# MiraPurkrabek/ProbPose_code

Hardware: AMD Instinct MI355X
Metric: person-crops/sec @ 256x192 bs64 (higher is better)
Workload: dtype f16x3; 1 GPU; ProbPose-small (ViT-S 12x384, 12 heads x 32) bs64 random 256x192 uint8 crops per GPU, flip_test=True, seeded random-init weights: preprocess -> backbone x2 passes -> ProbMapHead (heatmap branch + Sparsemax + 4 towers) -> ProbMap decode -> results in pinned host memory; crops_per_gpu=64, global_batch=64, parallelism=dp1, steps_in_flight=2

## Files before the change

include/probpose_mi355x.h:

```cpp
#ifndef PROBPOSE_MI355X_H_
#define PROBPOSE_MI355X_H_

#include <stddef.h>
#include <stdint.h>

#ifdef __cplusplus
extern "C" {
#endif

#define PP_ABI_VERSION 4


enum {
    PP_OK = 0,
    PP_ERR_INVALID_ARG = -1,
    PP_ERR_UNSUPPORTED = -2,
    PP_ERR_HIP = -3,
    PP_ERR_WORKSPACE = -4
};

#define PP_MAX_RADIUS 9
#define PP_MAX_TAPS (2 * PP_MAX_RADIUS + 1)

int pp_abi_version(void);
// ... 168 lines not shown
                         const float* head_b, float* logits_phased, int B, int H, int W, int Cin, int Cout, int K, void* stream);

int pp_probmap_head_decode_phased(const float* logits, const float* logits_flip, const int32_t* flip_indices,
                                  const double* taps, const int32_t* radius, int B, int K, int H, int W, double in_w,
                                  double in_h, float temperature, float normalize, float* avg_out, float* conv_out,
                                  float* locs, double* keypoints, float* scores, void* stream);

#define PP_DECODE_LOGITS 1
#define PP_DECODE_PHASED 2
#define PP_DECODE_SHIFT_HEATMAP 4
int pp_probmap_decode_flags(const float* maps, const float* maps_flip, const int32_t* flip_indices, const double* taps,
                            const int32_t* radius, int B, int K, int H, int W, double in_w, double in_h, float temperature,
                            float normalize, float* avg_out, float* conv_out, float* locs, double* keypoints, float* scores,
                            int flags, void* stream);

int pp_udp_heatmap_decode(const float* maps, const float* maps_flip, const int32_t* flip_indices, int B, int K, int H, int W,
                          double in_w, double in_h, int blur_kernel_size, float* avg_out, float* locs, double* keypoints,
                          float* scores, int flags, void* stream);

int pp_expmax_heatmap_decode(const float* maps, const float* maps_flip, const int32_t* flip_indices, const double* taps,
                             const int32_t* radius, int B, int K, int H, int W, double in_w, double in_h, float* avg_out,
                             float* conv_out, float* locs, double* keypoints, float* scores, int flags, void* stream);

int pp_argmax_probmap_decode(const float* logits, const float* logits_flip, const int32_t* flip_indices, int B, int K, int H, int W,
                             double in_w, double in_h, float temperature, float normalize, int blur_kernel_size, float* avg_out,
                             float* locs, double* keypoints, float* scores, int flags, void* stream);

int pp_conv3x3_splitk(int prec, const void* act_nhwc, const void* weight, float* partials, int B, int H, int W, int Cin,
                      int Cout, int groups, long long stride_act_g, long long stride_w_g, int ksplit, void* stream);
int pp_sum_maxpool_relu_nhwc(const float* partials, int nsplit, long long split_stride, const float* bias,
                             int images_per_group, void* out, int out_bf16, int N, int H, int W, int C, int ph, int pw,
                             void* stream);

long long pp_winograd_scratch_bytes(int B, int H, int W, int Cin);
int pp_conv3x3_winograd_maxpool_relu(const void* act_nhwc, const void* u_packed, const float* bias, void* v_scratch,
                                     void* out_pooled, int B, int H, int W, int Cin, int Cout, int pool_h, int pool_w, int groups,
                                     void* stream);

int pp_tower_final(const void* feat, int feat_bf16, const float* w, const float* bias,
                   const int32_t* flip_indices, float* out, int B, int passes, int C, int K, float err_div,
                   void* stream);

int pp_extended_oks(const double* gt_kpts, const double* gt_bbox, const double* gt_area, const double* dt_kpts,
                    const double* sigmas, const int* gt_visibilities, int G, int D, int K, int n_vis,
                    double confidence_thr, double padding, int use_area, int original, double* out, void* stream);

int pp_pack_records(const double* keypoints, const float* scores, const float* scalars, double* records, int n, void* stream);

int pp_revert_heatmaps_max(const float* heatmaps, const double* inverse_maps, float* out, int n, int K, int hm_h, int hm_w,
                           int img_h, int img_w, void* stream);

int pp_heatmap_posterior(float* heatmaps, const float* presence, double* scratch, int K, int H, int W, void* stream);

int pp_exoks_cells(const double* gt_kpts, const double* gt_bbox, const double* gt_area, const double* dt_kpts,
                   const double* sigmas, const int* gt_visibilities, const int* cell_gt_off, const int* cell_dt_off,
                   const long long* cell_out_off, int n_cells, int K, int n_vis, double confidence_thr, double padding,
                   int use_area, int original, double* out, void* stream);

int pp_exoks_match(const double* ious, const int* cell_gt_off, const int* cell_dt_off, const long long* cell_iou_off,
                   const unsigned char* gt_ignore, const unsigned char* gt_iscrowd, const double* gt_area,
                   const double* gt_bbox, const double* dt_area, const double* dt_bbox, const double* area_rng,
                   const double* iou_thrs, int n_cells, int max_gt_per_cell, int N_gt, int N_dt, int L, int A, int T,
                   int match_by_bbox, int* dt_match, unsigned char* dt_ignore, int* gt_match,
                   unsigned char* gt_ignore_out, double* sim_sum, int* sim_cnt, void* stream);

int pp_exmap_accumulate(const int* dt_match, const unsigned char* dt_ignore, const unsigned char* gt_ignore,
// ... 25 lines not shown
```

probpose_code_amd/_lib.py:

```python
import ctypes
import os
from ctypes import c_char_p, c_double, c_float, c_int, c_longlong, c_void_p

import torch

_HERE = os.path.dirname(os.path.abspath(__file__))
LIB_NAME = "libprobpose_mi355x.so"
LIB_PATH = os.path.join(_HERE, LIB_NAME)

PP_OK = 0
PP_ERR_INVALID_ARG = -1
PP_ERR_UNSUPPORTED = -2
PP_ERR_HIP = -3
PP_ERR_WORKSPACE = -4
PP_MAX_RADIUS = 9
PP_MAX_TAPS = 2 * PP_MAX_RADIUS + 1


class ProbPoseLibraryError(RuntimeError):

    def __init__(self, fn, status, message):
        super().__init__(f"{fn} failed with {status}: {message}")
        self.status = status

# ... 63 lines not shown
        c_int,
        [c_int, _P, _P, _P, _P, c_int, _P, c_int, c_int, c_int, c_int, c_int, c_int, c_int, c_int, c_int, c_float, _P],
    ),
    "pp_gemm_residual_layernorm": (
        c_int,
        [c_int, _P, _P, _P, _P, c_int, _P, _P, _P, c_float, _P, c_int, c_int, c_int, c_int, c_int, c_int, _P],
    ),
    "pp_gemm_residual_layernorm_ws": (
        c_int,
        [c_int, _P, _P, _P, _P, c_int, _P, _P, _P, c_float, _P, c_int, c_int, c_int, c_int, c_int, c_int, c_float, _P],
    ),
    "pp_mlp_residual_layernorm": (c_int, [_P, _P, _P, _P, _P, _P, _P, _P, _P, c_float, _P, c_int, c_int, c_int, _P]),
    "pp_proj_mlp_residual_layernorm": (
        c_int, [_P, _P, _P, _P, _P, _P, _P, _P, _P, _P, _P, _P, _P, c_float, _P, _P, _P, _P, c_int, c_int, c_int, _P]),
    "pp_vit_layer": (
        c_int, [_P, c_int, c_int, c_float, _P, _P, _P, _P, _P, _P, _P, _P, _P, _P, _P, _P, c_float, _P, _P, _P, _P, c_int, c_int,
                c_int, _P]),
    "pp_ffn_split_packed_bytes": (c_longlong, [c_int, c_int]),
    "pp_ffn_split_pack_weights": (c_int, [_P, _P, _P, c_int, c_int, _P]),
    "pp_ffn_split_residual_layernorm": (c_int, [_P, _P, _P, _P, _P, _P, _P, _P, c_float, _P, c_int, c_int, c_int, _P]),
    "pp_ffn_split_residual_layernorm_ws": (c_int, [_P, _P, _P, _P, _P, _P, _P, _P, c_float, _P, c_int, c_int, c_int, c_float, c_float, _P]),
    "pp_qkv_attention_split": (c_int, [_P, _P, _P, _P, c_int, c_int, c_int, c_int, c_float, _P]),
    "pp_qkv_attention_split_ws": (c_int, [_P, _P, _P, _P, c_int, c_int, c_int, c_int, c_float, c_float, _P]),
    "pp_qkv_attention_split_folded": (c_int, [_P] * 5 + [c_int] * 4 + [c_float, c_float, _P]),
    "pp_proj_split_packed_bytes": (c_longlong, [c_int]),
    "pp_proj_split_pack_weights": (c_int, [_P, _P, c_int, _P]),
    "pp_proj_ffn_split_residual_layernorm": (
        c_int, [_P, _P, _P, _P, _P, _P, _P, _P, _P, _P, _P, _P, _P, c_float, _P, c_int, c_int, c_int, _P]),
    "pp_proj_ffn_split_residual_layernorm_ws": (
        c_int, [_P, _P, _P, _P, _P, _P, _P, _P, _P, _P, _P, _P, _P, c_float, _P, c_int, c_int, c_int, c_float, c_float, c_float, _P]),
    "pp_proj_ffn_split_folded": (
        c_int, [_P] * 10 + [c_int, _P, c_int, _P, _P, _P, c_float, _P, _P, c_int, c_int, c_int, c_float, c_float, c_float, _P]),
    "pp_conv3x3_splitk": (c_int, [c_int, _P, _P, _P, c_int, c_int, c_int, c_int, c_int, c_int, c_longlong, c_longlong, c_int, _P]),
    "pp_sum_maxpool_relu_nhwc": (c_int, [_P, c_int, c_longlong, _P, c_int, _P, c_int, c_int, c_int, c_int, c_int, c_int, c_int, _P]),
    "pp_warp_affine_u8": (c_int, [_P, c_int, c_int, c_int, _P, _P, c_int, c_int, c_int, _P]),
    "pp_warp_affine_u8_batch": (c_int, [_P, _P, c_int, _P, _P, c_int, c_int, _P, c_int, c_int, c_int, _P]),
    "pp_extended_oks": (
        c_int, [_P, _P, _P, _P, _P, _P, c_int, c_int, c_int, c_int, c_double, c_double, c_int, c_int, _P, _P]),
    "pp_pack_records": (c_int, [_P, _P, _P, _P, c_int, _P]),
    "pp_revert_heatmaps_max": (c_int, [_P, _P, _P] + [c_int] * 6 + [_P]),
    "pp_heatmap_posterior": (c_int, [_P, _P, _P, c_int, c_int, c_int, _P]),
    "pp_exoks_cells": (
        c_int, [_P] * 9 + [c_int, c_int, c_int, c_double, c_double, c_int, c_int, _P, _P]),
    "pp_exoks_match": (
        c_int, [_P] * 12 + [c_int] * 8 + [_P] * 7),
    "pp_exmap_accumulate": (
        c_int, [_P] * 6 + [c_int] * 7 + [_P] * 5),
    "pp_conv_gemm": (
        c_int,
        [c_int, c_int, _P, _P, _P, _P, c_int, c_int, c_int, c_int, c_int, c_int, c_int, c_int,
         c_longlong, c_longlong, c_longlong, c_longlong, c_int, c_int, c_int, _P],
    ),
    "pp_attention": (c_int, [c_int, _P, _P, c_int, c_int, c_int, c_int, c_float, _P]),
    "pp_preproc_im2col": (c_int, [c_int, _P, c_int, _P, c_int, c_int, c_int, c_int, c_int, c_int, _P, _P, c_int, _P]),
    "pp_layernorm": (c_int, [_P, _P, _P, _P, c_int, c_int, c_float, c_int, _P]),
    "pp_maxpool_relu_nhwc": (c_int, [_P, c_int, _P, c_int, c_int, c_int, c_int, c_int, c_int, c_int, _P]),
    "pp_conv3x3_maxpool_relu": (c_int, [c_int, _P, _P, _P, _P, _P] + [c_int] * 8 + [c_longlong] * 3 + [c_int, _P]),
    "pp_winograd_scratch_bytes": (c_longlong, [c_int] * 4),
    "pp_conv3x3_winograd_maxpool_relu": (c_int, [_P] * 5 + [c_int] * 8 + [_P]),
    "pp_tower_final": (c_int, [_P, c_int, _P, _P, _P, _P, c_int, c_int, c_int, c_int, c_float, _P]),
    "pp_parea_scratch_bytes": (c_longlong, [c_int, c_int, c_int]),
    "pp_parea_thresholds": (c_int, [_P, c_int, c_int, c_int, _P, _P, _P, _P]),
    "pp_parea_compose": (c_int, [_P, c_int, c_int, c_int, c_int, _P, c_int, _P, _P, _P, c_int, _P, c_int, c_int, _P]),
    "pp_draw_poses": (
        c_int, [_P, c_int, c_int, _P, _P, _P, c_int, c_int, _P, _P, _P, c_int, c_double, c_float, c_float, c_float, _P, _P]),
    "pp_resize_bilinear_u8": (c_int, [_P, c_int, c_int, _P, c_int, c_int, _P]),
# ... 104 lines not shown
```

probpose_code_amd/csrc/pp_gemm.h:

```cpp
#pragma once
#include "pp_common.h"

namespace pp {

enum { G_LINEAR = 0, G_CONV3 = 1, G_DECONV = 2 };
enum { ACT_NONE = 0, ACT_GELU = 1, ACT_RELU = 2 };

struct GemmParams {
    const void* A;
    const void* W;
    void* C;
    const float* bias;
    const float* residual;
    int M, N, K;
    int lda, ldw, ldc;
    int H, Wd, Cin;
    int py, px;
    int act;
    int out_bf16;
    int gather;
    int res_mod;
    int ldres;
    const void* head_w;
    const float* head_b;
    float* head_out;
    int head_n;
    int ksplit;
    int groups;
    int pool_h, pool_w;
    int tap_inner;
    int tile_order;
    int planar_P;
    unsigned a_bytes, w_bytes;
    float w_inv = 1.0f;
    long long strideA_z, strideW_z, strideC_z, strideBias_z;
};

int gemm(const GemmParams& p, int prec, int groups, hipStream_t s);

bool panel_gemm_supported(const GemmParams& p, int prec, int groups);
int panel_gemm(const GemmParams& p, int groups, hipStream_t s);

bool conv_halo_supported(const GemmParams& p, int prec, int groups);
int conv_halo(const GemmParams& p, int groups, hipStream_t s);

bool panel_split_supported(const GemmParams& p, int prec, int groups);
int panel_split_gemm(const GemmParams& p, int prec, int groups, hipStream_t s);

bool linear_dma_supported(const GemmParams& p, int prec, int groups);
int linear_dma_gemm(const GemmParams& p, hipStream_t s);

}
```

probpose_code_amd/csrc/pp_gemm.hip:

```cpp
#include "pp_common.h"
#include "pp_gemm.h"
#include "pp_split.h"

#include <cstdlib>

namespace pp {

typedef __bf16 bf16x8 __attribute__((ext_vector_type(8)));
typedef __bf16 bf16x4 __attribute__((ext_vector_type(4)));
typedef float f32x4 __attribute__((ext_vector_type(4)));
typedef unsigned int u32x4 __attribute__((ext_vector_type(4)));
typedef __attribute__((address_space(3))) void* lds_ptr_t;

constexpr int BM = 128, BN = 128;
constexpr int GEMM_THREADS = 256;
constexpr int ROW_BYTES = 128;
constexpr int TILE_BYTES = BM * ROW_BYTES;
constexpr int BUF_BYTES = 2 * TILE_BYTES;
constexpr unsigned OOB_OFFSET = 0x7ffffff0u;

template <typename T>
struct Prec;
template <>
struct Prec<__bf16> {
// ... 496 lines not shown
}

extern "C" int pp_conv3x3_splitk(int prec, const void* act_nhwc, const void* weight, float* partials, int B, int H, int W,
                                 int Cin, int Cout, int groups, long long stride_act_g, long long stride_w_g, int ksplit,
                                 void* stream) {
    using namespace pp;
    PP_REQUIRE(act_nhwc && weight && partials, PP_ERR_INVALID_ARG, "pp_conv3x3_splitk: NULL argument");
    PP_REQUIRE(groups >= 1 && B > 0 && H > 0 && W > 0 && Cin > 0 && Cout > 0, PP_ERR_INVALID_ARG, "pp_conv3x3_splitk: bad shape");
    PP_REQUIRE(ksplit >= 1 && ksplit <= 16 && (ksplit == 1 || ksplit == 3 || ksplit == 9 || Cin % (32 * ksplit) == 0), PP_ERR_UNSUPPORTED,
               "pp_conv3x3_splitk: ksplit must be 1, 3 or 9 (whole taps), or a count of channel ranges (Cin % (32 ksplit) == 0, split-fp16 wide-tile kernel)");
    GemmParams p{};
    p.A = act_nhwc; p.W = weight; p.C = partials; p.bias = nullptr; p.residual = nullptr;
    p.M = B * H * W; p.N = Cout;
    p.K = 9 * Cin / ksplit;
    p.lda = Cin; p.ldw = 9 * Cin; p.ldc = Cout;
    p.H = H; p.Wd = W; p.Cin = Cin;
    p.act = ACT_NONE; p.out_bf16 = 0; p.gather = G_CONV3; p.ldres = Cout;
    p.ksplit = ksplit;
    const size_t esz = prec == PP_PREC_BF16 ? 2 : 4;
    const size_t ab = (size_t)B * H * W * Cin * esz, wb = (size_t)Cout * 9 * Cin * esz;
    PP_REQUIRE(ab < 0x7ffffff0u && wb < 0x7ffffff0u, PP_ERR_UNSUPPORTED, "pp_conv3x3_splitk: operands must be smaller than 2 GiB");
    p.a_bytes = (unsigned)ab; p.w_bytes = (unsigned)wb;
    p.strideA_z = stride_act_g; p.strideW_z = stride_w_g; p.strideC_z = (long long)p.M * Cout; p.strideBias_z = 0;
    if (ksplit != 1 && ksplit != 3 && ksplit != 9) {
        PP_REQUIRE(panel_enabled() && panel_split_supported(p, prec, groups * ksplit), PP_ERR_UNSUPPORTED,
                   "pp_conv3x3_splitk: this slice count is a channel-range split, built for the split-fp16 wide-tile kernel only (use pp_conv3x3_splitk_slices)");
        return panel_split_gemm(p, prec, groups * ksplit, reinterpret_cast<hipStream_t>(stream));
    }
    if (panel_enabled() && panel_gemm_supported(p, prec, groups * ksplit))
        return panel_gemm(p, groups * ksplit, reinterpret_cast<hipStream_t>(stream));
    return gemm(p, prec, groups * ksplit, reinterpret_cast<hipStream_t>(stream));
}

extern "C" int pp_deconv_head(const void* act_nhwc, const void* weight, const float* bias, const void* head_w,
                              const float* head_b, float* logits_phased, int B, int H, int W, int Cin, int Cout, int K,
                              void* stream) {
    using namespace pp;
    PP_REQUIRE(act_nhwc && weight && head_w && head_b && logits_phased, PP_ERR_INVALID_ARG, "pp_deconv_head: NULL argument");
    PP_REQUIRE(B > 0 && H > 0 && W > 0 && Cin > 0, PP_ERR_INVALID_ARG, "pp_deconv_head: bad shape");
    PP_REQUIRE(Cout == 256 && K >= 1 && K <= 28 && Cin % 32 == 0 && (4 * Cin) % 128 == 0 && (H * W) % 4 == 0, PP_ERR_UNSUPPORTED,
               "pp_deconv_head: built for 256 deconvolution channels, at most 28 output maps, Cin % 32 == 0, H*W % 4 == 0");
    GemmParams p{};
    p.A = act_nhwc; p.W = weight; p.C = logits_phased; p.bias = bias; p.residual = nullptr;
    p.M = B * H * W; p.N = Cout; p.K = 4 * Cin;
    p.lda = Cin; p.ldw = p.K; p.ldc = Cout;
    p.H = H; p.Wd = W; p.Cin = Cin; p.py = -1; p.px = -1;
    p.act = ACT_RELU; p.out_bf16 = 1; p.gather = G_DECONV; p.ldres = Cout;
    p.head_w = head_w; p.head_b = head_b; p.head_out = logits_phased; p.head_n = K;
    const size_t ab = (size_t)B * H * W * Cin * 2, wb = (size_t)Cout * p.K * 2;
    PP_REQUIRE(ab < 0x7ffffff0u && wb < 0x7ffffff0u, PP_ERR_UNSUPPORTED, "pp_deconv_head: operands must be smaller than 2 GiB");
    p.a_bytes = (unsigned)ab; p.w_bytes = (unsigned)wb;
    p.strideA_z = 0; p.strideW_z = (long long)Cout * 4 * Cin; p.strideC_z = 0; p.strideBias_z = 0;
    return panel_gemm(p, 4, reinterpret_cast<hipStream_t>(stream));
}

extern "C" int pp_deconv_head_split(const void* act_nhwc, const void* weight, const float* bias, const void* head_w_packed,
                                    const float* head_b, float* logits_phased, int B, int H, int W, int Cin, int Cout, int K,
                                    void* stream) {
    using namespace pp;
    PP_REQUIRE(act_nhwc && weight && head_w_packed && head_b && logits_phased, PP_ERR_INVALID_ARG, "pp_deconv_head_split: NULL argument");
    PP_REQUIRE(B > 0 && H > 0 && W > 0 && Cin > 0, PP_ERR_INVALID_ARG, "pp_deconv_head_split: bad shape");
    PP_REQUIRE(Cout == 256 && K >= 1 && K <= 28 && Cin % 32 == 0, PP_ERR_UNSUPPORTED,
               "pp_deconv_head_split: built for 256 deconvolution channels, at most 28 output maps, Cin % 32 == 0");
    GemmParams p{};
    p.A = act_nhwc; p.W = weight; p.C = logits_phased; p.bias = bias; p.residual = nullptr;
    p.M = B * H * W; p.N = Cout; p.K = 4 * Cin;
// ... 13 lines not shown
```

probpose_code_amd/engine.py:

```python
import math
import os
import warnings
from typing import Dict, Optional, Sequence

import numpy as np
import ctypes

import torch

from . import _lib
from .codecs import oks_kernel_taps
from .weights import PackedWeights, from_split, pack, to_split

PREC = {"bf16": 0, "f32": 1, "f16x3": 2}
_DTYPE = {"bf16": torch.bfloat16, "f32": torch.float32, "f16x3": torch.float32}
_FMT = {"bf16": 1, "f32": 0, "f16x3": 2}
ACT_NONE, ACT_GELU, ACT_RELU = 0, 1, 2
CONV3X3, DECONV = 1, 2


PLAN_DEFAULTS = dict(fuse_mlp=True, fuse_proj=True, fuse_qkv=True, split_k=True, fuse_attn=True, fuse_head=True, fuse_resln=None,
                     fuse_pool=True, fuse_qkv_attn=True, winograd=True, ln_fold=True, small_plan=True, head_two_streams=True)
SMALL_PLAN_ROWS_BELOW = 6912


def plan_from_env() -> Dict[str, object]:
    out: Dict[str, object] = {}
    for k in PLAN_DEFAULTS:
        v = os.environ.get("PP_" + k.upper())
        if v in ("0", "1"):
            out[k] = v == "1"
    return out


class _CapturedGraph:

    def __init__(self, graph, static_in, out, events, side_stream, raw_stream):
        self.graph, self.static_in, self.out, self.events, self.side_stream, self.raw_stream = graph, static_in, out, events, side_stream, raw_stream

    def release(self):
        if self.graph is None and self.raw_stream is None:
            return
        try:
            if torch.cuda.is_available():
                torch.cuda.synchronize()
        except Exception:
            pass
        self.graph = None
        self.out = self.static_in = None
        self.events = []
        self.side_stream = None
        raw, self.raw_stream = self.raw_stream, None
        if raw:
            try:
                _lib.lib.pp_stream_destroy(ctypes.c_void_p(raw))
# ... 113 lines not shown
        self.ln_fold = bool(precision == "f16x3" and pl["ln_fold"] and not self._proj_packed and not self._ffn_packed
                            and self.w.has("l0.fc1.wf") and self.E % 192 == 0 and self.w.ffn_dims % 192 == 0)
        self.ln_fold_fused = bool(precision == "f16x3" and pl["ln_fold"] and self.fuse_qkv_attn and self._proj_packed and self.w.has("l1.qkv.wf")
                                  and (self.w.ffn_dims // 128) % 2 == 0 and self.w.num_layers >= 2)
        if precision == "f16x3":
            if self.fuse_qkv_attn and self._proj_packed:
                self.layer_plan = "two launches per layer (pp_qkv_attention_split + pp_proj_ffn_split_residual_layernorm)"
                if self.ln_fold_fused:
                    self.layer_plan += "; ln1 of layers 1 .. L - 1 folded into the qkv projection (pp_proj_ffn_split_folded -> pp_qkv_attention_split_folded)"
            elif self._proj_packed:
                self.layer_plan = "three launches per layer (pp_gemm qkv + pp_attention + pp_proj_ffn_split_residual_layernorm)"
            else:
                self.layer_plan = "generic (pp_gemm / pp_attention / pp_layernorm per layer)"
                if self.ln_fold:
                    self.layer_plan += ("; from the row count at which the twelve-wave Linear kernel engages: LayerNorm folded into the Linear "
                                        "layers (pp_linear_ln_folded x4 + pp_attention per layer, residual stream in the operand format)")
                if self.hd == 80:
                    self.layer_plan += "; attention at head dim 80: pp_attention_hd80.hip (the q . k contraction zero-padded to 96 on chip)"
                if self._small_at(1):
                    self.layer_plan += (f"; batches of fewer than {SMALL_PLAN_ROWS_BELOW} token rows: the small-batch plan (pp_skinny_linear x4 + "
                                        "pp_attention per layer, LayerNorm in the Linear launches)")
                elif self.small_plan and self.E > 1024:
                    self.layer_plan += f"; no small-batch plan at E = {self.E} (pp_skinny_linear's LayerNorm tail ends at 1024 columns): this plan at every batch size"
            if pl["fuse_qkv_attn"] and not self.fuse_qkv_attn and self.E == 384 and self.hd == 32:
                warnings.warn(
                    f"ProbPoseEngine: {self.Np}-token sequences ({img_size[0]}x{img_size[1]} input) miss the fused qkv + attention kernel, "
                    f"which is built for 192 tokens (256x192); this model runs {self.layer_plan}", RuntimeWarning, stacklevel=2)
        else:
            self.layer_plan = "bf16 / f32 plan"
        self.winograd = (precision == "f16x3" and pl["winograd"] and self.w.has("tower0.wino")
                         and _lib.lib.pp_winograd_scratch_bytes(1, self.Hp, self.Wp, self.E) > 0)
        if self.w.has("tower0.wino") and not self.winograd:
            self.w.t.pop("tower0.wino")
        self._logits_phased = False
        self._head_stream: Optional[torch.cuda.Stream] = None
        self._capture_events: list = []
        self._eager_events: dict = {}
        self.profile: Optional[Dict[str, list]] = None
        self.stage_hook = None
        self.pools = ((4, 3), (2, 2), (2, 2))
        hs, ws_ = self.Hp, self.Wp
        self.tower_hw = []
        for ph, pw_ in self.pools if self.head_kind == "probmap" else ():
            self.tower_hw.append((hs, ws_))
            hs, ws_ = hs // ph, ws_ // pw_
        if self.head_kind == "probmap" and (hs, ws_) != (1, 1):
            raise ValueError(
                f"scalar towers reduce the {self.Hp}x{self.Wp} feature map to {hs}x{ws_}; the reference "
                "reshapes them to (B, 1, K) (probmap_head.py:780-783), which needs 1x1"
            )

    def ksplit(self, nb: int, th: int, tw: int) -> int:
        return int(_lib.lib.pp_conv3x3_splitk_slices(self.prec, int(nb), int(th), int(tw), self.E, self.E, 4))

    def _workspace(self, B: int, passes: int, slot: int = 0) -> Dict[str, torch.Tensor]:
        self._check_options()
        key = (B, passes, slot)
        if key in self._ws:
            return self._ws[key]
        dev, T, f32 = self.device, self.dtype, torch.float32
        nb = B * passes
        M = nb * self.Np
        E, Fd = self.E, self.w.ffn_dims
        dc = self.w.deconv_channels
        shape = _lib.PlanShape(prec=self.prec, n_img=nb, n_tokens=self.Np, embed=E, ffn=Fd, patch_k=3 * self.P * self.P, n_keypoints=self.K,
                               feat_h=self.Hp, feat_w=self.Wp, heat_h=self.Hh, heat_w=self.Wh, deconv_channels=dc[0] if dc else 0)
# ... 273 lines not shown
                    and ww % 4 == 0 and self.K <= 28 and nb * hh * ww * 4 >= 192 * 192):
                self._call("deconv_head", "pp_deconv_head_split", src.data_ptr(), wj.data_ptr(), w[f"deconv{j}.b"].data_ptr(),
                           w["final.w_head"].data_ptr(), w["final.b"].data_ptr(), ws["logits"].data_ptr(), nb, hh, ww, cin, cout,
                           self.K, st)
                self._logits_phased = True
                return ws["logits"]
            if ob == 2 and self._small_at(nb * self.Np) and nb * hh * ww <= 1536 and cin % 32 == 0 and cout % 32 == 0:
                self._call("deconv", "pp_skinny_deconv", src.data_ptr(), wj.data_ptr(), w[f"deconv{j}.b"].data_ptr(), dst.data_ptr(), nb, hh, ww, cin,
                           cout, st)
                src, cin, hh, ww = dst, cout, hh * 2, ww * 2
                continue
            self._call("deconv", "pp_conv_gemm", self.prec, DECONV, src.data_ptr(), wj.data_ptr(),
                       w[f"deconv{j}.b"].data_ptr(), dst.data_ptr(), nb, hh, ww, cin, cout, -1, -1, 1, 0, 0, 0, 0, cout,
                       ACT_RELU, ob, st)
            src, cin, hh, ww = dst, cout, hh * 2, ww * 2
        P = hh * ww
        if ob == 2 and self._small_at(nb * self.Np) and cin % 64 == 0 and self._final_padded is not None:
            wp, bp = self._final_padded
            self._call("final_conv", "pp_skinny_conv1x1_planar", src.data_ptr(), wp.data_ptr(), bp.data_ptr(), ws["logits"].data_ptr(), nb, P, cin, self.K,
                       w.inv("final.w"), st)
            return ws["logits"]
        self._gemm(st, src, w["final.w"], w["final.b"], ws["logits"], nb * P, self.K, cin, planar=P, out_bf16=0)
        return ws["logits"]

    def towers(self, feat: torch.Tensor, B: int, passes: int, flip_indices, ws, st) -> torch.Tensor:
        w, E = self.w, self.E
        nb = B * passes
        ob = self.fmt
        src, stride_src = feat, 0
        for j, (th, tw) in enumerate(self.tower_hw):
            ph, pw_ = self.pools[j]
            out = ws[f"t{j}"]
            rows = nb * th * tw
            if self.split_k and f"tp{j}" in ws:
                part = ws[f"tp{j}"]
                ks = part.shape[0]
                self._call("conv3x3_splitk", "pp_conv3x3_splitk", self.prec, src.data_ptr(), w[f"tower{j}.w"].data_ptr(),
                           part.data_ptr(), nb, th, tw, E, E, 4, stride_src, E * 9 * E, ks, st)
                self._call("maxpool", "pp_sum_maxpool_relu_nhwc", part.data_ptr(), ks, 4 * rows * E, w[f"tower{j}.b"].data_ptr(),
                           nb, ws[f"p{j}"].data_ptr(), ob, 4 * nb, th, tw, E, ph, pw_, st)
                src = ws[f"p{j}"]
                stride_src = nb * (th // ph) * (tw // pw_) * E
                continue
            if j == 0 and self.winograd and ws.get("wino") is not None and stride_src == 0 and (ph, pw_) == (4, 3):
                self._call("conv3x3", "pp_conv3x3_winograd_maxpool_relu", src.data_ptr(), w["tower0.wino"].data_ptr(), w["tower0.b"].data_ptr(),
                           ws["wino"].data_ptr(), ws["p0"].data_ptr(), nb, th, tw, E, E, ph, pw_, 4, st)
            elif self.fuse_pool:
                self._call("conv3x3", "pp_conv3x3_maxpool_relu", self.prec, src.data_ptr(), w[f"tower{j}.w"].data_ptr(),
                           w[f"tower{j}.b"].data_ptr(), ws[f"p{j}"].data_ptr(), out.data_ptr(), nb, th, tw, E, E, ph, pw_, 4,
                           stride_src, E * 9 * E, E, ob, st)
            else:
                self._call("conv3x3", "pp_conv_gemm", self.prec, CONV3X3, src.data_ptr(), w[f"tower{j}.w"].data_ptr(),
                           w[f"tower{j}.b"].data_ptr(), out.data_ptr(), nb, th, tw, E, E, 0, 0, 4, stride_src,
                           E * 9 * E, nb * th * tw * E, E, E, ACT_NONE, ob, st)
                self._call("maxpool", "pp_maxpool_relu_nhwc", out.data_ptr(), ob, ws[f"p{j}"].data_ptr(), ob, 4 * nb, th, tw, E, ph,
                           pw_, st)
            src = ws[f"p{j}"]
            stride_src = nb * (th // ph) * (tw // pw_) * E
        fi = self._flip_indices(flip_indices) if passes == 2 else None
        self._call("tower_final", "pp_tower_final", src.data_ptr(), ob, w["tower_out.w"].data_ptr(), w["tower_out.b"].data_ptr(),
                  _lib.ptr(fi), ws["scalars"].data_ptr(), B, passes, E, self.K, 1.0, st)
        return ws["scalars"]

    def _check_imgs(self, imgs: torch.Tensor):
        assert imgs.dim() == 4 and imgs.is_cuda, "expects a (B,3,H,W) tensor on the GPU"
        assert imgs.dtype in (torch.uint8, torch.float32), "crops are uint8 (raw) or float32 (already preprocessed)"
# ... 232 lines not shown
```

probpose_code_amd/weights.py:

```python
import math
from dataclasses import dataclass, field
from typing import Dict, List

import torch

TOWERS = ("probability", "visibility", "oks", "error")
BN_EPS = 1e-5


def to_split(x: torch.Tensor) -> torch.Tensor:
    K = x.shape[-1]
    assert K % 32 == 0, f"split-fp16 tensors need a last dimension that is a multiple of 32, got {K}"
    x = x.float()
    hi = x.half()
    lo = (x - hi.float()).half()
    lead = x.shape[:-1]
    blocks = torch.stack([hi.reshape(*lead, K // 32, 32), lo.reshape(*lead, K // 32, 32)], dim=-2)
    return blocks.reshape(*lead, 2 * K).contiguous().view(torch.float32)


def from_split(c: torch.Tensor) -> torch.Tensor:
    K = c.shape[-1]
    v = c.contiguous().view(torch.float16).reshape(*c.shape[:-1], K // 32, 2, 32).float()
    return (v[..., 0, :] + v[..., 1, :]).reshape(c.shape)
# ... 93 lines not shown
        return k in self.t


def _bn_fold(sd, name):
    scale = sd[name + ".weight"].float() / torch.sqrt(sd[name + ".running_var"].float() + BN_EPS)
    shift = sd[name + ".bias"].float() - sd[name + ".running_mean"].float() * scale
    return scale, shift


def pack_head_split(w32: torch.Tensor) -> torch.Tensor:
    assert tuple(w32.shape) == (32, 256)
    w32 = w32.float()
    hi = w32.half()
    lo = (w32 - hi.float()).half()
    lane = torch.arange(64)
    fr, fg = lane % 16, lane // 16
    j = torch.arange(8)
    ch_in_blk = torch.where(j < 4, 4 * fg[:, None] + j[None, :], 16 + 4 * fg[:, None] + (j[None, :] - 4))
    out = torch.empty((4, 2, 2, 2, 64, 8), dtype=torch.float16)
    for cg in range(4):
        for kb in range(2):
            ch = 64 * cg + 32 * kb + ch_in_blk
            for nf in range(2):
                rows = (16 * nf + fr)[:, None].expand(64, 8)
                out[cg, kb, nf, 0] = hi[rows, ch]
                out[cg, kb, nf, 1] = lo[rows, ch]
    return out.reshape(-1).view(torch.float32).contiguous()


def winograd_weights(w: torch.Tensor) -> torch.Tensor:
    G = torch.tensor([[1.0, 0.0, 0.0], [0.5, 0.5, 0.5], [0.5, -0.5, 0.5], [0.0, 0.0, 1.0]], dtype=torch.float64)
    u = torch.einsum("ai,ocij,bj->aboc", G, w.double(), G)
    return u.reshape(16, w.shape[0], w.shape[1]).float()


def pack(sd: Dict[str, torch.Tensor], dtype: torch.dtype, device, split: bool = False, scale_linear: bool = True,
         num_heads: int = 0, fold_ln: bool = True) -> PackedWeights:
    sd = {k: v.detach().cpu() for k, v in normalize_state_dict(sd).items()}
    if split and scale_linear and num_heads > 0:
        n_layers = 1 + max(int(k.split(".")[2]) for k in sd if k.startswith("backbone.layers."))
        for i in range(n_layers):
            if sd[f"backbone.layers.{i}.attn.qkv.weight"].shape[1] % num_heads == 0:
                balance_attention_dims(sd, f"backbone.layers.{i}.", num_heads)
    f32 = lambda x: x.float().contiguous().to(device)
    inv_scale: Dict[str, float] = {}
    if split:
        def op(x, name="weights", scaled=False):
            check_split_range(name, x)
            x = x.float()
            if scaled and scale_linear:
                e = weight_scale_exponent(x)
                x = x * 2.0 ** e
                inv_scale[name] = 2.0 ** -e
            return to_split(x.contiguous()).to(device)
    else:
        op = lambda x, name=None, scaled=False: x.float().contiguous().to(dtype).to(device)
    pw = sd["backbone.patch_embed.projection.weight"]
    E = pw.shape[0]
    L = 1 + max(int(k.split(".")[2]) for k in sd if k.startswith("backbone.layers."))
    Fd = sd["backbone.layers.0.ffn.layers.0.0.weight"].shape[0]
    K = sd["head.final_layer.weight"].shape[0]
    t: Dict[str, torch.Tensor] = {}
    t["patch_w"] = op(pw.reshape(E, -1), "patch_w")
    t["patch_b"] = f32(sd["backbone.patch_embed.projection.bias"])
    t["pos_embed"] = f32(sd["backbone.pos_embed"].reshape(-1, E))
    for i in range(L):
# ... 28 lines not shown
    t["ln_f.w"] = f32(sd["backbone.ln1.weight"])
    t["ln_f.b"] = f32(sd["backbone.ln1.bias"])

    deconv_channels = []
    j = 0
    while f"head.deconv_layers.{3 * j}.weight" in sd:
        w = sd[f"head.deconv_layers.{3 * j}.weight"].float()
        assert w.shape[2:] == (4, 4), "only deconv kernel 4 / stride 2 / pad 1 (the ProbPose config) is packed"
        scale, shift = _bn_fold(sd, f"head.deconv_layers.{3 * j + 1}")
        w = w * scale.view(1, -1, 1, 1)
        cin, cout = w.shape[:2]
        ph = torch.empty((2, 2, cout, 4 * cin))
        for py in range(2):
            for px in range(2):
                for ty in range(2):
                    for tx in range(2):
                        tap = ty * 2 + tx
                        ph[py, px, :, tap * cin : (tap + 1) * cin] = w[:, :, 3 - 2 * ty - py, 3 - 2 * tx - px].t()
        t[f"deconv{j}.w"] = op(ph, f"deconv{j}.w")
        t[f"deconv{j}.b"] = f32(shift)
        deconv_channels.append(cout)
        j += 1
    t["final.w"] = op(sd["head.final_layer.weight"].reshape(K, -1), "final.w")
    t["final.b"] = f32(sd["head.final_layer.bias"])
    if K <= 32:
        wpad = torch.zeros((32, t["final.w"].shape[1]), dtype=torch.float32)
        wpad[:K] = sd["head.final_layer.weight"].reshape(K, -1).float()
        t["final.w_pad"] = op(wpad, "final.w_pad")
        if split and wpad.shape[1] == 256:
            t["final.w_head"] = pack_head_split(wpad).to(device)

    head_kind = "probmap" if any(k.startswith(f"head.{TOWERS[0]}_layers.") for k in sd) else "heatmap"
    for c in range(3 if head_kind == "probmap" else 0):
        ws, bs, wino = [], [], []
        for tw in TOWERS:
            base = f"head.{tw}_layers."
            w = sd[base + f"{4 * c}.weight"].float()
            b = sd[base + f"{4 * c}.bias"].float()
            scale, shift = _bn_fold(sd, base + f"{4 * c + 1}")
            w = w * scale.view(-1, 1, 1, 1)
            ws.append(w.permute(0, 2, 3, 1).reshape(w.shape[0], -1))
            bs.append(b * scale + shift)
            if c == 0 and split:
                wino.append(winograd_weights(w))
        if c == 0 and split and w.shape[1] % 128 == 0 and w.shape[0] % 96 == 0:
            t["tower0.wino"] = op(torch.stack(wino), "tower0.wino")
        t[f"tower{c}.w"] = op(torch.stack(ws), f"tower{c}.w")
        t[f"tower{c}.b"] = f32(torch.stack(bs))
    if head_kind == "probmap":
        t["tower_out.w"] = f32(torch.stack([sd[f"head.{tw}_layers.12.weight"].float().reshape(K, -1) for tw in TOWERS]))
        t["tower_out.b"] = f32(torch.stack([sd[f"head.{tw}_layers.12.bias"].float() for tw in TOWERS]))
    return PackedWeights(dtype=dtype, embed_dims=E, num_layers=L, ffn_dims=Fd, num_keypoints=K,
                         deconv_channels=deconv_channels, t=t, inv_scale=inv_scale, head_kind=head_kind)
```

Before: 15010 crops/s.

## Lower 2x2 tower conv to dense GEMM via new split-K ring linear kernel

After: 15070 crops/s (median of 6 runs). Within noise of the previous version (+0.4%).

```diff
diff --git a/include/probpose_mi355x.h b/include/probpose_mi355x.h
--- a/include/probpose_mi355x.h
+++ b/include/probpose_mi355x.h
@@ -224,6 +224,10 @@
                              int images_per_group, void* out, int out_bf16, int N, int H, int W, int C, int ph, int pw,
                              void* stream);
 
+int pp_linear_splitk_slices(int M, int N, int K, int groups);
+int pp_linear_splitk(int prec, const void* act, const void* weight, float* partials, int M, int N, int K, int groups,
+                     long long stride_act_g, long long stride_w_g, int ksplit, float w_inv_scale, void* stream);
+
 long long pp_winograd_scratch_bytes(int B, int H, int W, int Cin);
 int pp_conv3x3_winograd_maxpool_relu(const void* act_nhwc, const void* u_packed, const float* bias, void* v_scratch,
                                      void* out_pooled, int B, int H, int W, int Cin, int Cout, int pool_h, int pool_w, int groups,
diff --git a/probpose_code_amd/_lib.py b/probpose_code_amd/_lib.py
--- a/probpose_code_amd/_lib.py
+++ b/probpose_code_amd/_lib.py
@@ -119,6 +119,8 @@
     "pp_proj_ffn_split_folded": (
         c_int, [_P] * 10 + [c_int, _P, c_int, _P, _P, _P, c_float, _P, _P, c_int, c_int, c_int, c_float, c_float, c_float, _P]),
     "pp_conv3x3_splitk": (c_int, [c_int, _P, _P, _P, c_int, c_int, c_int, c_int, c_int, c_int, c_longlong, c_longlong, c_int, _P]),
+    "pp_linear_splitk_slices": (c_int, [c_int] * 4),
+    "pp_linear_splitk": (c_int, [c_int, _P, _P, _P, c_int, c_int, c_int, c_int, c_longlong, c_longlong, c_int, c_float, _P]),
     "pp_sum_maxpool_relu_nhwc": (c_int, [_P, c_int, c_longlong, _P, c_int, _P, c_int, c_int, c_int, c_int, c_int, c_int, c_int, _P]),
     "pp_warp_affine_u8": (c_int, [_P, c_int, c_int, c_int, _P, _P, c_int, c_int, c_int, _P]),
     "pp_warp_affine_u8_batch": (c_int, [_P, _P, c_int, _P, _P, c_int, c_int, _P, c_int, c_int, c_int, _P]),
diff --git a/probpose_code_amd/csrc/pp_gemm.h b/probpose_code_amd/csrc/pp_gemm.h
--- a/probpose_code_amd/csrc/pp_gemm.h
+++ b/probpose_code_amd/csrc/pp_gemm.h
@@ -50,4 +50,7 @@
 bool linear_dma_supported(const GemmParams& p, int prec, int groups);
 int linear_dma_gemm(const GemmParams& p, hipStream_t s);
 
+bool linear_splitk_ring_supported(const GemmParams& p, int prec, int groups);
+int linear_splitk_ring(const GemmParams& p, int groups, hipStream_t s);
+
 }
diff --git a/probpose_code_amd/csrc/pp_gemm.hip b/probpose_code_amd/csrc/pp_gemm.hip
--- a/probpose_code_amd/csrc/pp_gemm.hip
+++ b/probpose_code_amd/csrc/pp_gemm.hip
@@ -552,6 +552,44 @@
     return gemm(p, prec, groups * ksplit, reinterpret_cast<hipStream_t>(stream));
 }
 
+extern "C" int pp_linear_splitk_slices(int M, int N, int K, int groups) {
+    if (M <= 0 || N <= 0 || K <= 0 || groups <= 0) return 1;
+    const long long tiles = (long long)((M + 127) / 128) * ((N + 127) / 128) * groups;
+    int ks = 1;
+    while (ks < 4 && tiles * (2 * ks) <= 512 && K % (32 * 2 * ks) == 0) ks *= 2;
+    return ks;
+}
+
+extern "C" int pp_linear_splitk(int prec, const void* act, const void* weight, float* partials, int M, int N, int K, int groups,
+                                long long stride_act_g, long long stride_w_g, int ksplit, float w_inv_scale, void* stream) {
+    using namespace pp;
+    PP_REQUIRE(act && weight && partials, PP_ERR_INVALID_ARG, "pp_linear_splitk: NULL argument");
+    PP_REQUIRE(groups >= 1 && M > 0 && N > 0 && K > 0 && stride_act_g >= 0 && stride_w_g >= 0, PP_ERR_INVALID_ARG, "pp_linear_splitk: bad shape");
+    PP_REQUIRE(prec == PP_PREC_F16X3, PP_ERR_UNSUPPORTED, "pp_linear_splitk: built for PP_PREC_F16X3 (the other modes keep pp_conv3x3_splitk)");
+    PP_REQUIRE(ksplit >= 1 && ksplit <= 16 && K % (32 * ksplit) == 0, PP_ERR_UNSUPPORTED,
+               "pp_linear_splitk: K must be a multiple of ksplit K-blocks of 32 elements, ksplit 1 .. 16");
+    PP_REQUIRE(N % 4 == 0, PP_ERR_UNSUPPORTED, "pp_linear_splitk: N must be a multiple of 4");
+    {
+        unsigned u;
+        __builtin_memcpy(&u, &w_inv_scale, 4);
+        PP_REQUIRE((u >> 31) == 0 && (u & 0x007fffffu) == 0 && ((u >> 23) & 0xffu) >= 127 - 40 && ((u >> 23) & 0xffu) <= 127 + 40, PP_ERR_INVALID_ARG,
+                   "pp_linear_splitk: the weight scale must be a power of two in [2^-40, 2^40]");
+    }
+    GemmParams p{};
+    p.w_inv = w_inv_scale;
+    p.A = act; p.W = weight; p.C = partials; p.bias = nullptr; p.residual = nullptr;
+    p.M = M; p.N = N;
+    p.K = K / ksplit;
+    p.lda = K; p.ldw = K; p.ldc = N;
+    p.act = ACT_NONE; p.out_bf16 = 0; p.gather = G_LINEAR; p.ldres = N;
+    p.ksplit = ksplit;
+    const size_t ab = (size_t)M * K * 4, wb = (size_t)N * K * 4;
+    PP_REQUIRE(ab < 0x7ffffff0u && wb < 0x7ffffff0u, PP_ERR_UNSUPPORTED, "pp_linear_splitk: operands must be smaller than 2 GiB");
+    p.a_bytes = (unsigned)ab; p.w_bytes = (unsigned)wb;
+    p.strideA_z = stride_act_g; p.strideW_z = stride_w_g; p.strideC_z = (long long)M * N; p.strideBias_z = 0;
+    return linear_splitk_ring(p, groups * ksplit, reinterpret_cast<hipStream_t>(stream));
+}
+
 extern "C" int pp_deconv_head(const void* act_nhwc, const void* weight, const float* bias, const void* head_w,
                               const float* head_b, float* logits_phased, int B, int H, int W, int Cin, int Cout, int K,
                               void* stream) {
diff --git a/probpose_code_amd/csrc/pp_linear_ring.hip b/probpose_code_amd/csrc/pp_linear_ring.hip
--- /dev/null
+++ b/probpose_code_amd/csrc/pp_linear_ring.hip
@@ -0,0 +1,149 @@
+#include "pp_common.h"
+#include "pp_gemm.h"
+#include "pp_split.h"
+
+namespace pp {
+namespace lring {
+
+typedef float f32x4 __attribute__((ext_vector_type(4)));
+typedef unsigned int u32x4 __attribute__((ext_vector_type(4)));
+typedef __attribute__((address_space(3))) void* lds_ptr_t;
+
+constexpr int BM = 128, BN = 128, BK = 32, THREADS = 256;
+constexpr int ROW_BYTES = 128;
+constexpr int TILE_BYTES = BM * ROW_BYTES;
+constexpr int STAGE = 2 * TILE_BYTES;
+constexpr int NST = 4;
+constexpr int NI = 8;
+constexpr unsigned OOB_OFFSET = 0x7ffffff0u;
+
+__device__ __forceinline__ int swz(int row, int chunk) { return row * ROW_BYTES + ((chunk ^ (row & 7)) << 4); }
+
+template <int N>
+__device__ __forceinline__ void wait_vm_lgkm() {
+    __builtin_amdgcn_s_waitcnt((N & 15) | (7 << 4) | (0 << 8) | ((N >> 4) << 14));
+}
+
+__global__ __launch_bounds__(THREADS, 1) void linear_splitk_ring_kernel(const GemmParams p) {
+    extern __shared__ __attribute__((aligned(16))) char smem[];
+    const int tid = threadIdx.x, lane = tid & 63, wave = tid >> 6;
+    const int wy = wave >> 1, wx = wave & 1;
+    const int f_row = lane & 15, f_kg = lane >> 4;
+
+    const int ntn = (p.N + BN - 1) / BN, ntm = (p.M + BM - 1) / BM;
+    const int tiles_per_group = ntn * ntm, ntiles = tiles_per_group * p.groups;
+    const int nk = p.K / BK;
+    int t = blockIdx.x;
+    if ((ntiles & 7) == 0) t = (t & 7) * (ntiles >> 3) + (t >> 3);
+    const int z = t / tiles_per_group, r = t - z * tiles_per_group;
+    const int n0 = (r % ntn) * BN, m0 = (r / ntn) * BM;
+    const int problems = p.groups / p.ksplit;
+    const int zp = z % problems, zs = z / problems;
+
+    const size_t k_off = (size_t)zs * p.K * 4;
+    const char* Act = reinterpret_cast<const char*>(p.A) + (size_t)zp * p.strideA_z * 4 + k_off;
+    const char* Wt = reinterpret_cast<const char*>(p.W) + (size_t)zp * p.strideW_z * 4 + k_off;
+    const __amdgpu_buffer_rsrc_t a_rsrc = __builtin_amdgcn_make_buffer_rsrc(const_cast<char*>(Act), 0, p.a_bytes - (unsigned)k_off, 0x00020000);
+    const __amdgpu_buffer_rsrc_t w_rsrc = __builtin_amdgcn_make_buffer_rsrc(const_cast<char*>(Wt), 0, p.w_bytes - (unsigned)k_off, 0x00020000);
+
+    const int d_row = lane >> 3;
+    const unsigned d_chunk_bytes = (unsigned)(((lane & 7) ^ d_row) << 4);
+    unsigned a_voff[4], w_voff[4];
+#pragma unroll
+    for (int j = 0; j < 4; ++j) {
+        const int rr = wave * 32 + j * 8 + d_row;
+        const int n = n0 + rr, m = m0 + rr;
+        w_voff[j] = n < p.N ? (unsigned)n * (unsigned)(p.ldw * 4) + d_chunk_bytes : OOB_OFFSET;
+        a_voff[j] = m < p.M ? (unsigned)m * (unsigned)(p.lda * 4) + d_chunk_bytes : OOB_OFFSET;
+    }
+    auto stage = [&](int kt, int buf) {
+        const unsigned kb = (unsigned)(kt * BK * 4);
+        char* wdst = smem + buf * STAGE + wave * 4096;
+        char* adst = wdst + TILE_BYTES;
+#pragma unroll
+        for (int j = 0; j < 4; ++j) {
+            const unsigned wv = w_voff[j] == OOB_OFFSET ? OOB_OFFSET : w_voff[j] + kb;
+            __builtin_amdgcn_raw_ptr_buffer_load_lds(w_rsrc, (lds_ptr_t)(wdst + j * 1024), 16, wv, 0, 0, 0);
+            const unsigned av = a_voff[j] == OOB_OFFSET ? OOB_OFFSET : a_voff[j] + kb;
+            __builtin_amdgcn_raw_ptr_buffer_load_lds(a_rsrc, (lds_ptr_t)(adst + j * 1024), 16, av, 0, 0, 0);
+        }
+    };
+
+#pragma unroll
+    for (int s = 0; s < NST - 1; ++s)
+        if (s < nk) stage(s, s);
+
+    f32x4 acc[4][4];
+#pragma unroll
+    for (int i = 0; i < 4; ++i)
+#pragma unroll
+        for (int j = 0; j < 4; ++j) acc[i][j] = f32x4{0.f, 0.f, 0.f, 0.f};
+
+    int buf = 0;
+    for (int kt = 0; kt < nk; ++kt) {
+        const int ahead = (kt + NST - 1 < nk ? kt + NST - 1 : nk) - (kt + 1);
+        __builtin_amdgcn_sched_barrier(0);
+        if (ahead >= 2) wait_vm_lgkm<2 * NI>();
+        else if (ahead == 1) wait_vm_lgkm<NI>();
+        else wait_vm_lgkm<0>();
+        __builtin_amdgcn_s_barrier();
+        asm volatile("" ::: "memory");
+        __builtin_amdgcn_sched_barrier(0);
+        if (kt + NST - 1 < nk) stage(kt + NST - 1, buf == 0 ? NST - 1 : buf - 1);
+        const char* wbase = smem + buf * STAGE;
+        const char* abase = wbase + TILE_BYTES;
+        u32x4 fwh[4], fwl[4], fah[4], fal[4];
+#pragma unroll
+        for (int f = 0; f < 4; ++f) {
+            fwh[f] = *reinterpret_cast<const u32x4*>(wbase + swz(wy * 64 + f * 16 + f_row, f_kg));
+            fwl[f] = *reinterpret_cast<const u32x4*>(wbase + swz(wy * 64 + f * 16 + f_row, 4 + f_kg));
+            fah[f] = *reinterpret_cast<const u32x4*>(abase + swz(wx * 64 + f * 16 + f_row, f_kg));
+            fal[f] = *reinterpret_cast<const u32x4*>(abase + swz(wx * 64 + f * 16 + f_row, 4 + f_kg));
+        }
+#pragma unroll
+        for (int nf = 0; nf < 4; ++nf)
+#pragma unroll
+            for (int mf = 0; mf < 4; ++mf)
+                acc[nf][mf] = split_mma(__builtin_bit_cast(f16x8, fwh[nf]), __builtin_bit_cast(f16x8, fwl[nf]),
+                                        __builtin_bit_cast(f16x8, fah[mf]), __builtin_bit_cast(f16x8, fal[mf]), acc[nf][mf]);
+        asm volatile("" ::: "memory");
+        buf = buf + 1 == NST ? 0 : buf + 1;
+    }
+
+    float* __restrict__ C = reinterpret_cast<float*>(p.C) + (size_t)z * p.strideC_z;
+#pragma unroll
+    for (int mf = 0; mf < 4; ++mf) {
+        const int m = m0 + wx * 64 + mf * 16 + f_row;
+        if (m >= p.M) continue;
+#pragma unroll
+        for (int nf = 0; nf < 4; ++nf) {
+            const int n = n0 + wy * 64 + nf * 16 + f_kg * 4;
+            if (n < p.N) *reinterpret_cast<f32x4*>(C + (size_t)m * p.ldc + n) = acc[nf][mf] * p.w_inv;
+        }
+    }
+}
+
+}
+
+bool linear_splitk_ring_supported(const GemmParams& p, int prec, int groups) {
+    return prec == PP_PREC_F16X3 && p.gather == G_LINEAR && p.ksplit >= 1 && groups % p.ksplit == 0 && p.K > 0 && p.K % lring::BK == 0 &&
+           p.lda % 32 == 0 && p.ldw % 32 == 0 && p.strideA_z % 32 == 0 && p.strideW_z % 32 == 0 && p.N % 4 == 0 && p.ldc % 4 == 0 &&
+           p.out_bf16 == 0 && !p.bias && !p.residual && p.planar_P == 0 && p.act == ACT_NONE && p.a_bytes < lring::OOB_OFFSET &&
+           p.w_bytes < lring::OOB_OFFSET;
+}
+
+int linear_splitk_ring(const GemmParams& p_in, int groups, hipStream_t s) {
+    using namespace lring;
+    GemmParams p = p_in;
+    p.groups = groups;
+    PP_REQUIRE(linear_splitk_ring_supported(p, PP_PREC_F16X3, groups), PP_ERR_UNSUPPORTED, "pp linear ring: shape outside what the kernel was built for");
+    const long long ntiles = (long long)((p.N + BN - 1) / BN) * ((p.M + BM - 1) / BM) * groups;
+    PP_REQUIRE(ntiles < (1ll << 30), PP_ERR_UNSUPPORTED, "pp linear ring: too many output tiles");
+    constexpr int lds = NST * STAGE;
+    PP_HIP_CHECK(hipFuncSetAttribute(reinterpret_cast<const void*>(linear_splitk_ring_kernel), hipFuncAttributeMaxDynamicSharedMemorySize, lds));
+    hipLaunchKernelGGL(linear_splitk_ring_kernel, dim3((unsigned)ntiles), dim3(THREADS), lds, s, p);
+    PP_LAUNCH_CHECK();
+    return PP_OK;
+}
+
+}
diff --git a/probpose_code_amd/engine.py b/probpose_code_amd/engine.py
--- a/probpose_code_amd/engine.py
+++ b/probpose_code_amd/engine.py
@@ -20,7 +20,7 @@
 
 
 PLAN_DEFAULTS = dict(fuse_mlp=True, fuse_proj=True, fuse_qkv=True, split_k=True, fuse_attn=True, fuse_head=True, fuse_resln=None,
-                     fuse_pool=True, fuse_qkv_attn=True, winograd=True, ln_fold=True, small_plan=True, head_two_streams=True)
+                     fuse_pool=True, fuse_qkv_attn=True, winograd=True, ln_fold=True, small_plan=True, head_two_streams=True, tower_dense=True)
 SMALL_PLAN_ROWS_BELOW = 6912
 
 
@@ -200,6 +200,9 @@
                          and _lib.lib.pp_winograd_scratch_bytes(1, self.Hp, self.Wp, self.E) > 0)
         if self.w.has("tower0.wino") and not self.winograd:
             self.w.t.pop("tower0.wino")
+        self.tower_dense = bool(precision == "f16x3" and pl["tower_dense"] and pl["split_k"] and self.w.has("tower2.dense"))
+        if self.w.has("tower2.dense") and not self.tower_dense:
+            self.w.t.pop("tower2.dense")
         self._logits_phased = False
         self._head_stream: Optional[torch.cuda.Stream] = None
         self._capture_events: list = []
@@ -539,6 +542,17 @@
             ph, pw_ = self.pools[j]
             out = ws[f"t{j}"]
             rows = nb * th * tw
+            if self.tower_dense and j == 2 and (th, tw, ph, pw_) == (2, 2, 2, 2) and f"tp{j}" in ws and not self._small_at(nb * self.Np):
+                ks = int(_lib.lib.pp_linear_splitk_slices(nb, 4 * E, 4 * E, 4))
+                part = ws[f"tp{j}"]
+                assert ks * 4 * rows * E <= part.numel()
+                self._call("conv3x3_splitk", "pp_linear_splitk", self.prec, src.data_ptr(), w["tower2.dense"].data_ptr(), part.data_ptr(),
+                           nb, 4 * E, 4 * E, 4, stride_src, 16 * E * E, ks, w.inv("tower2.dense"), st)
+                self._call("maxpool", "pp_sum_maxpool_relu_nhwc", part.data_ptr(), ks, 4 * rows * E, w[f"tower{j}.b"].data_ptr(),
+                           nb, ws[f"p{j}"].data_ptr(), ob, 4 * nb, th, tw, E, ph, pw_, st)
+                src = ws[f"p{j}"]
+                stride_src = nb * (th // ph) * (tw // pw_) * E
+                continue
             if self.split_k and f"tp{j}" in ws:
                 part = ws[f"tp{j}"]
                 ks = part.shape[0]
diff --git a/probpose_code_amd/weights.py b/probpose_code_amd/weights.py
--- a/probpose_code_amd/weights.py
+++ b/probpose_code_amd/weights.py
@@ -149,6 +149,15 @@
     G = torch.tensor([[1.0, 0.0, 0.0], [0.5, 0.5, 0.5], [0.5, -0.5, 0.5], [0.0, 0.0, 1.0]], dtype=torch.float64)
     u = torch.einsum("ai,ocij,bj->aboc", G, w.double(), G)
     return u.reshape(16, w.shape[0], w.shape[1]).float()
+
+
+def dense_2x2_weights(w: torch.Tensor) -> torch.Tensor:
+    co, ci = w.shape[:2]
+    d = torch.empty((4, co, 4, ci), dtype=w.dtype)
+    for q in range(4):
+        for r in range(4):
+            d[q, :, r, :] = w[:, :, r // 2 - q // 2 + 1, r % 2 - q % 2 + 1]
+    return d.reshape(4 * co, 4 * ci)
 
 
 def pack(sd: Dict[str, torch.Tensor], dtype: torch.dtype, device, split: bool = False, scale_linear: bool = True,
@@ -243,7 +252,7 @@
 
     head_kind = "probmap" if any(k.startswith(f"head.{TOWERS[0]}_layers.") for k in sd) else "heatmap"
     for c in range(3 if head_kind == "probmap" else 0):
-        ws, bs, wino = [], [], []
+        ws, bs, wino, dense = [], [], [], []
         for tw in TOWERS:
             base = f"head.{tw}_layers."
             w = sd[base + f"{4 * c}.weight"].float()
@@ -254,6 +263,10 @@
             bs.append(b * scale + shift)
             if c == 0 and split:
                 wino.append(winograd_weights(w))
+            if c == 2 and split and w.shape[0] == w.shape[1] and w.shape[0] % 32 == 0 and w.shape[0] <= 512:
+                dense.append(dense_2x2_weights(w))
+        if dense:
+            t["tower2.dense"] = op(torch.stack(dense), "tower2.dense", scaled=True)
         if c == 0 and split and w.shape[1] % 128 == 0 and w.shape[0] % 96 == 0:
             t["tower0.wino"] = op(torch.stack(wino), "tower0.wino")
         t[f"tower{c}.w"] = op(torch.stack(ws), f"tower{c}.w")
```
